# BadgerTechnologies/navigation

Measured on AMD Instinct MI355X. Metric: scored trajectories/sec (whole node) + costmap inflation cells/sec, 400x400 map, higher is better.
Workload: dtype f64

## Files before the change

navigation_amd/csrc/navgpu_fleet.h:

```cpp
#pragma once
#include <algorithm>
#include <cfloat>
#include <cmath>
#include <cstdio>
#include <cstdlib>
#include <cstring>
#include <ctime>
#include <mutex>
#include <string>
#include <vector>

#include "navgpu_device.h"

using namespace navgpu;

namespace navgpu {
extern thread_local std::string g_last_error;

#define HIP_TRY(expr)                                                                              \
  do {                                                                                             \
    hipError_t e_ = (expr);                                                                        \
    if (e_ != hipSuccess) {                                                                        \
      g_last_error = std::string(#expr) + ": " + hipGetErrorString(e_);                            \
      return NAVGPU_ERR_HIP;                                                                       \
    }                                                                                              \
  } while (0)

inline hipError_t waitStream(hipStream_t s) { return hipStreamSynchronize(s); }

struct EventPair {
  int kernel;
  hipEvent_t a, b;
};
int ensureCompleteGrids(navgpu_fleet* f, uint32_t first, uint32_t count);
}

struct navgpu_fleet {
  navgpu_fleet_desc desc{};
  std::recursive_mutex mu;
  hipStream_t stream = nullptr;
  CostmapDev cm{};
  PlannerDev pl{};
  bool planner_configured = false, inflation_configured = false, planner_staged = false;
  bool shift_pending = false;
  uint32_t shift_first = 0, shift_count = 0;
  std::vector<void*> allocs;
  std::vector<double> h_origin;
  std::vector<double> h_fp_spec;
  std::vector<uint32_t> h_fp_n;
  navgpu_inflation_params infl{};
  navgpu_obstacle_params obsp{};
  double fp_radius = 0.0;
  std::vector<void*> pinned;
  ObsCsr* hp_obs = nullptr;
  uint32_t *hp_cnt = nullptr, *hp_used = nullptr, *hp_plan_cnt = nullptr;
  float* hp_pts = nullptr;
  double *hp_fpw = nullptr, *hp_pose = nullptr, *hp_plan = nullptr, *hp_front = nullptr;
  int32_t *hp_shift = nullptr, *hp_align = nullptr;
  uint32_t *hp_reach = nullptr, *hp_fpn = nullptr;
  uint8_t *cm_stage_dev = nullptr, *cm_stage_host = nullptr, *pl_stage_dev = nullptr, *pl_stage_host = nullptr;
  size_t cm_stage_bytes = 0, pl_stage_bytes = 0;
  bool bounded_grids = true;
  std::vector<uint8_t> grid_partial;
  std::vector<int32_t> h_box;
  std::vector<uint64_t> inputs_gen, cycle_gen;
  void touchInputs(uint32_t first, uint32_t count) {
    for (uint32_t i = first; i < first + count && i < inputs_gen.size(); ++i) ++inputs_gen[i];
  }
  navgpu_robot_state* hp_state = nullptr;
  navgpu_plan_result* hp_result = nullptr;
  bool hp_dma_pending = false;
  int cycles_in_flight = 1;
  int res_slot = 0;
  hipEvent_t ev_cycle[2] = {nullptr, nullptr}, ev_cm_h2d = nullptr, ev_pl_h2d = nullptr;
  bool ev_cycle_set[2] = {false, false}, ev_cm_set = false, ev_pl_set = false;
  hipError_t waitMirrors(hipEvent_t ev, bool set) {
    if (cycles_in_flight < 2) return navgpu::waitStream(stream);
    return set ? hipEventSynchronize(ev) : hipSuccess;
  }
  struct LocalPlannerState {
    std::vector<double> plan;
    double T[3] = {0, 0, 0};
    bool has_T = false, have_plan = false;
    bool xy_tolerance_latch = false, rotating_to_goal = false;
  };
  std::vector<LocalPlannerState> lp;
  navgpu_local_limits lp_limits{};
  bool lp_configured = false;
  struct TpHost {
    std::vector<double> plan;
    double final_goal_x = 0, final_goal_y = 0;
    bool final_goal_position_valid = false;
    navgpu_tp_state st{};
    std::vector<navgpu_tp_sample> made;
    int n_points = 0;
  };
  TpDev tp{};
  bool tp_configured = false;
// ... 38 lines not shown
    return NAVGPU_OK;
  }
  template <class T>
  int allocPinned(T** p, size_t count) {
    void* q = nullptr;
    hipError_t e = hipHostMalloc(&q, std::max<size_t>(count * sizeof(T), 16), hipHostMallocDefault);
    if (e != hipSuccess) {
      g_last_error = std::string("hipHostMalloc: ") + hipGetErrorString(e);
      return NAVGPU_ERR_HIP;
    }
    memset(q, 0, std::max<size_t>(count * sizeof(T), 16));
    pinned.push_back(q);
    *p = static_cast<T*>(q);
    return NAVGPU_OK;
  }
  void release(void* q) {
    if (!q) return;
    auto it = std::find(allocs.begin(), allocs.end(), q);
    if (it != allocs.end()) allocs.erase(it);
    hipFree(q);
  }
  bool rangeOk(uint32_t first, uint32_t count) const { return count > 0 && first < desc.n_instances && count <= desc.n_instances - first; }

  int beginKernel(int k, EventPair* ep) {
    if (!profiling || !((prof_mask >> k) & 1u)) return NAVGPU_OK;
    if (free_events.empty()) {
      EventPair n{};
      HIP_TRY(hipEventCreate(&n.a));
      HIP_TRY(hipEventCreate(&n.b));
      free_events.push_back(n);
    }
    *ep = free_events.back();
    free_events.pop_back();
    ep->kernel = k;
    HIP_TRY(hipEventRecord(ep->a, stream));
    return NAVGPU_OK;
  }
  int endKernel(EventPair* ep) {
    if (!profiling || !ep->a) return NAVGPU_OK;
    HIP_TRY(hipEventRecord(ep->b, stream));
    events.push_back(*ep);
    if (events.size() > 8192) return foldEvents();
    return NAVGPU_OK;
  }
  int foldEvents() {
    if (events.empty()) return NAVGPU_OK;
    HIP_TRY(waitStream(stream));
    for (auto& e : events) {
      float ms = 0;
      HIP_TRY(hipEventElapsedTime(&ms, e.a, e.b));
      prof_ms[e.kernel] += ms;
      prof_n[e.kernel] += 1;
      free_events.push_back(e);
    }
    events.clear();
    return NAVGPU_OK;
  }
};

#ifndef NAVGPU_TEST_NO_FLEET_LOCK
struct FleetGuard {
  std::lock_guard<std::recursive_mutex> lk;
  explicit FleetGuard(navgpu_fleet* f) : lk(f->mu) { (void)hipSetDevice(f->desc.device); }
};
#else
struct FleetGuard {
  explicit FleetGuard(navgpu_fleet* f) { (void)hipSetDevice(f->desc.device); }
};
#endif

#define PROFILED(fleet, kid, launch_expr)            \
  do {                                               \
    EventPair ep_{};                                 \
    int rc_ = (fleet)->beginKernel((kid), &ep_);     \
    if (rc_) return rc_;                             \
    launch_expr;                                     \
    rc_ = (fleet)->endKernel(&ep_);                  \
    if (rc_) return rc_;                             \
  } while (0)

inline int checkLaunch() {
  hipError_t e = hipGetLastError();
  if (e != hipSuccess) {
    g_last_error = std::string("kernel launch: ") + hipGetErrorString(e);
    return NAVGPU_ERR_HIP;
  }
  return NAVGPU_OK;
}
```

navigation_amd/csrc/navgpu_host.cpp:

```cpp
#include "navgpu_fleet.h"

namespace navgpu {
thread_local std::string g_last_error;
}

extern "C" {

const char* navgpu_version(void) { return "navgpu 0.1 (gfx950)"; }
const char* navgpu_strerror(int status) {
  switch (status) {
    case NAVGPU_OK: return "ok";
    case NAVGPU_ERR_INVALID: return "invalid argument";
    case NAVGPU_ERR_NO_DEVICE: return "no usable HIP device (this library has no CPU fallback)";
    case NAVGPU_ERR_HIP: return "HIP runtime error";
    case NAVGPU_ERR_CAPACITY: return "input exceeds a capacity given at fleet creation";
    case NAVGPU_ERR_STATE: return "call sequence violated";
    default: return "unknown status";
  }
}
const char* navgpu_last_error(void) { return g_last_error.c_str(); }
int navgpu_device_count(void) {
  int n = 0;
  if (hipGetDeviceCount(&n) != hipSuccess) return 0;
  return n;
// ... 7 lines not shown
  if (!d || !out || d->n_instances == 0 || d->size_x == 0 || d->size_y == 0 || !(d->resolution > 0)) return NAVGPU_ERR_INVALID;
  if ((uint64_t)((d->size_x + 127) / 128) * ((d->size_y + 15) / 16) > 8192) {
    g_last_error = "navgpu_fleet_create: costmap larger than 16.7 M cells";
    return NAVGPU_ERR_CAPACITY;
  }
  if (d->max_footprint > (uint32_t)kMaxFootprint) return NAVGPU_ERR_CAPACITY;
  if ((uint64_t)d->size_x * d->size_y > (1ull << 30) || d->size_x > 65535 || d->size_y > 65535) return NAVGPU_ERR_CAPACITY;
  int ndev = 0;
  if (hipGetDeviceCount(&ndev) != hipSuccess || ndev <= 0 || d->device < 0 || d->device >= ndev) {
    g_last_error = "no HIP device";
    return NAVGPU_ERR_NO_DEVICE;
  }
  HIP_TRY(hipSetDevice(d->device));
  auto* f = new navgpu_fleet();
  f->desc = *d;
  if (f->desc.max_observations == 0) f->desc.max_observations = 1;
  if (f->desc.max_points == 0) f->desc.max_points = 1;
  if (f->desc.max_plan == 0) f->desc.max_plan = 1;
  if (f->desc.max_sim_steps == 0) f->desc.max_sim_steps = 64;
  const uint32_t n = d->n_instances;
  if (hipStreamCreateWithFlags(&f->stream, hipStreamNonBlocking) != hipSuccess) {
    g_last_error = "hipStreamCreate failed";
    delete f;
    return NAVGPU_ERR_NO_DEVICE;
  }
  CostmapDev& cm = f->cm;
  cm.nx = d->size_x;
  cm.ny = d->size_y;
  cm.cells = d->size_x * d->size_y;
  cm.cells_padded = (cm.cells + 63) & ~63u;
  cm.res = d->resolution;
  cm.layers = d->layers;
  cm.track_unknown = d->track_unknown;
  cm.master_default = d->track_unknown ? kNoInfo : kFree;
  cm.obstacle_default = d->track_unknown ? kNoInfo : kFree;
  cm.obs_enabled = 1;
  cm.footprint_clearing = 1;
  cm.combination_method = 1;
  cm.max_obstacle_height = 2.0;
  cm.z_voxels = 10;
  cm.unknown_threshold = 15;
  cm.mark_threshold = 0;
  cm.origin_z = 0.0;
  cm.z_resolution = 0.2;
  cm.max_obs = f->desc.max_observations;
  cm.max_points = f->desc.max_points;
// ... 81 lines not shown
  pl.inv_res = 1.0 / cm.res;
  pl.origin = cm.origin;
  pl.master = cm.master;
  pl.max_plan = f->desc.max_plan;
  pl.max_sim_steps = f->desc.max_sim_steps;
  {
    size_t off = 0;
    auto take = [&](size_t bytes) {
      const size_t at = off;
      off = (off + bytes + 255) & ~(size_t)255;
      return at;
    };
    const size_t o_state = take(sizeof(navgpu_robot_state) * n), o_front = take(sizeof(double) * 2 * n), o_align = take(sizeof(int32_t) * n),
                 o_reach = take(sizeof(uint32_t) * n), o_pcnt = take(sizeof(uint32_t) * n), o_plan = take(sizeof(double) * 2 * (size_t)n * pl.max_plan);
    f->pl_stage_bytes = off;
    uint8_t *d = nullptr, *h = nullptr;
    A(d, off);
    if ((rc = f->allocPinned(&h, off)) != 0) {
      navgpu_fleet_destroy(f);
      return rc;
    }
    f->pl_stage_dev = d;
    f->pl_stage_host = h;
    pl.state = reinterpret_cast<navgpu_robot_state*>(d + o_state);
    pl.front_last = reinterpret_cast<double*>(d + o_front);
    pl.align_on = reinterpret_cast<int32_t*>(d + o_align);
    pl.bfs_reach = reinterpret_cast<uint32_t*>(d + o_reach);
    pl.plan_count = reinterpret_cast<uint32_t*>(d + o_pcnt);
    pl.plan = reinterpret_cast<double*>(d + o_plan);
    f->hp_state = reinterpret_cast<navgpu_robot_state*>(h + o_state);
    f->hp_front = reinterpret_cast<double*>(h + o_front);
    f->hp_align = reinterpret_cast<int32_t*>(h + o_align);
    f->hp_reach = reinterpret_cast<uint32_t*>(h + o_reach);
    f->hp_plan_cnt = reinterpret_cast<uint32_t*>(h + o_pcnt);
    f->hp_plan = reinterpret_cast<double*>(h + o_plan);
  }
  A(pl.fp_spec, (size_t)n * kMaxFootprint * 2);
  A(pl.fp_n, n);
  A(pl.axis_count, (size_t)n * 4);
  A(pl.path, (size_t)n * pl.cells);
  A(pl.goal, (size_t)n * pl.cells);
  A(pl.goal_front, (size_t)n * pl.cells);
  if (bfs_scratch_words(cm.nx, cm.ny)) A(pl.bfs_scratch, (size_t)n * bfs_scratch_words(cm.nx, cm.ny));
  pl.bfs_grids = 3;
  pl.within = nullptr;
  A(pl.bfs_box, (size_t)n * 8);
// ... 23 lines not shown
  for (auto& s : st) {
    memset(&s, 0, sizeof(s));
    s.last_min_x = -FLT_MAX;
    s.last_min_y = -FLT_MAX;
    s.last_max_x = FLT_MAX;
    s.last_max_y = FLT_MAX;
  }
  hipError_t e = hipMemcpyAsync(cm.state, st.data(), sizeof(InstCostmapState) * n, hipMemcpyHostToDevice, f->stream);
  if (e == hipSuccess) e = hipMemsetAsync(pl.bfs_reach, 0, sizeof(uint32_t) * n, f->stream);
  if (e == hipSuccess) e = hipMemsetAsync(pl.bfs_levels, 0, sizeof(uint32_t) * 3 * n, f->stream);
  if (e == hipSuccess) e = waitStream(f->stream);
  if (e != hipSuccess || checkLaunch() != NAVGPU_OK) {
    if (e != hipSuccess) g_last_error = std::string("fleet init: ") + hipGetErrorString(e);
    navgpu_fleet_destroy(f);
    return NAVGPU_ERR_NO_DEVICE;
  }
  *out = f;
  return NAVGPU_OK;
}

int navgpu_fleet_destroy(navgpu_fleet* f) {
  if (!f) return NAVGPU_ERR_INVALID;
  if (f->stream) waitStream(f->stream);
  for (auto& e : f->events) {
    hipEventDestroy(e.a);
    hipEventDestroy(e.b);
  }
  for (auto& e : f->free_events) {
    hipEventDestroy(e.a);
    hipEventDestroy(e.b);
  }
  for (hipEvent_t e : {f->ev_cycle[0], f->ev_cycle[1], f->ev_cm_h2d, f->ev_pl_h2d})
    if (e) hipEventDestroy(e);
  for (void* p : f->allocs) hipFree(p);
  for (void* p : f->pinned) hipHostFree(p);
  if (f->stream) hipStreamDestroy(f->stream);
  delete f;
  return NAVGPU_OK;
}
int navgpu_sync(navgpu_fleet* f) {
  if (!f) return NAVGPU_ERR_INVALID;
  FleetGuard guard_(f);
  HIP_TRY(waitStream(f->stream));
  return NAVGPU_OK;
}
void* navgpu_stream(navgpu_fleet* f) { return f ? (void*)f->stream : nullptr; }
int navgpu_fleet_set_alloc_limit(navgpu_fleet* f, uint64_t max_bytes) {
  if (!f) return NAVGPU_ERR_INVALID;
  FleetGuard guard_(f);
  f->alloc_limit = (size_t)max_bytes;
  return NAVGPU_OK;
}

int navgpu_fleet_set_origin(navgpu_fleet* f, uint32_t first, uint32_t count, const double* xy) {
  if (!f || !xy || !f->rangeOk(first, count)) return NAVGPU_ERR_INVALID;
  FleetGuard guard_(f);
  f->touchInputs(first, count);
  memcpy(&f->h_origin[(size_t)first * 2], xy, sizeof(double) * 2 * count);
// ... 492 lines not shown
  if (e == hipSuccess) e = hipMemcpyAsync(f->pl.fp_n + first, &fp_n[first], sizeof(uint32_t) * count, hipMemcpyHostToDevice, f->stream);
  if (e == hipSuccess) e = waitStream(f->stream);
  if (e != hipSuccess) {
    if (fresh_prep) f->release(fresh_prep);
    g_last_error = std::string("navgpu_set_footprint: ") + hipGetErrorString(e);
    return NAVGPU_ERR_HIP;
  }
  f->h_fp_n.swap(fp_n);
  f->h_fp_spec.swap(fp_spec);
  f->fp_radius = fp_radius;
  if (f->planner_configured) {
    uint8_t* keep = fresh_prep ? fresh_prep : f->pl.prep;
    if (fresh_prep) f->release(f->pl.prep);
    f->pl = np;
    f->pl.prep = keep;
    f->pl.prep_stride = stride;
  }
  return NAVGPU_OK;
}

int navgpu_costmap_stage(navgpu_fleet* f, uint32_t first, uint32_t count, const double* poses, const navgpu_observation* obs,
                         uint32_t n_obs, const float* points, uint32_t n_points_total) {
  if (!f || !poses || !f->rangeOk(first, count) || (n_obs && (!obs || (!points && n_points_total)))) return NAVGPU_ERR_INVALID;
  FleetGuard guard_(f);
  CostmapDev& cm = f->cm;
  if (f->desc.rolling_window && f->shift_pending) return NAVGPU_ERR_STATE;
  if (f->desc.rolling_window) f->touchInputs(first, count);
  HIP_TRY(f->waitMirrors(f->ev_cm_h2d, f->ev_cm_set));
  for (uint32_t li = 0; li < count; ++li) f->hp_cnt[first + li] = f->hp_used[first + li] = 0;
  for (uint32_t k = 0; k < n_obs; ++k) {
    const navgpu_observation& o = obs[k];
    if (o.instance < first || o.instance >= first + count) return NAVGPU_ERR_INVALID;
    const uint32_t i = o.instance;
    if (f->hp_cnt[i] >= cm.max_obs || f->hp_used[i] + o.n_points > cm.max_points) return NAVGPU_ERR_CAPACITY;
    if ((uint64_t)o.first_point + o.n_points > n_points_total) return NAVGPU_ERR_INVALID;
    ObsCsr& d = f->hp_obs[(size_t)i * cm.max_obs + f->hp_cnt[i]++];
    d.first_point = f->hp_used[i];
    d.n_points = o.n_points;
    d.flags = o.flags;
    d.pad = 0;
    d.ox = o.origin_x;
    d.oy = o.origin_y;
    d.oz = o.origin_z;
    d.obstacle_range = o.obstacle_range;
    d.raytrace_range = o.raytrace_range;
    if (o.n_points)
      memcpy(&f->hp_pts[((size_t)i * cm.max_points + f->hp_used[i]) * 3], points + (size_t)o.first_point * 3, sizeof(float) * 3 * o.n_points);
// ... 50 lines not shown

static int applyPendingShift(navgpu_fleet* f, uint32_t first, uint32_t count) {
  CostmapDev& cm = f->cm;
  if (!(f->desc.rolling_window && f->shift_pending)) return NAVGPU_OK;
  if (first != f->shift_first || count != f->shift_count) return NAVGPU_ERR_STATE;
  if (first != 0 || count != f->desc.n_instances) return NAVGPU_ERR_INVALID;
  launch_shift_u8(cm.master, cm.master_alt, cm, first, count, cm.master_default, f->stream);
  std::swap(cm.master, cm.master_alt);
  f->pl.master = cm.master;
  if (cm.obst) {
    launch_shift_u8(cm.obst, cm.obst_alt, cm, first, count, cm.obstacle_default, f->stream);
    std::swap(cm.obst, cm.obst_alt);
  }
  if (cm.voxel) {
    launch_shift_u32(cm.voxel, cm.voxel_alt, cm, first, count, 0x0000FFFFu, f->stream);
    std::swap(cm.voxel, cm.voxel_alt);
  }
  f->shift_pending = false;
  return NAVGPU_OK;
}

int navgpu_costmap_update(navgpu_fleet* f, uint32_t first, uint32_t count) {
  if (!f || !f->rangeOk(first, count)) return NAVGPU_ERR_INVALID;
  FleetGuard guard_(f);
  f->touchInputs(first, count);
  CostmapDev& cm = f->cm;
  if ((cm.layers & NAVGPU_LAYER_INFLATION) && !f->inflation_configured) return NAVGPU_ERR_STATE;
  {
    int rc = applyPendingShift(f, first, count);
    if (rc) return rc;
  }
  PROFILED(f, NAVGPU_K_OBSTACLE, launch_obstacle(cm, first, count, nullptr, 0, f->stream));
  PROFILED(f, NAVGPU_K_MERGE, launch_merge(cm, first, count, nullptr, f->stream));
  if (cm.layers & NAVGPU_LAYER_INFLATION) PROFILED(f, NAVGPU_K_INFLATE, launch_inflate(cm, first, count, nullptr, f->stream));
  return checkLaunch();
}

int navgpu_costmap_bounds(navgpu_fleet* f, uint32_t first, uint32_t count, int32_t* boxes) {
  if (!f || !boxes || !f->rangeOk(first, count)) return NAVGPU_ERR_INVALID;
  FleetGuard guard_(f);
  std::vector<InstCostmapState> st(count);
  HIP_TRY(hipMemcpyAsync(st.data(), f->cm.state + first, sizeof(InstCostmapState) * count, hipMemcpyDeviceToHost, f->stream));
  HIP_TRY(waitStream(f->stream));
  for (uint32_t i = 0; i < count; ++i)
    for (int k = 0; k < 4; ++k) boxes[4 * i + k] = st[i].box[k];
  return NAVGPU_OK;
}
// ... 79 lines not shown
extern "C++" int navgpu::ensureCompleteGrids(navgpu_fleet* f, uint32_t first, uint32_t count) {
  if (NAVGPU_DEBUG_ENV("NAVGPU_DEBUG_RAW_GRIDS")) return NAVGPU_OK;
  for (uint32_t i = first; i < first + count; ++i)
    if (f->grid_partial[i] && f->cycle_gen[i] != f->inputs_gen[i]) {
      g_last_error = "MapGrids of instance " + std::to_string(i) + " were searched inside the robot's box only and the costmap / plan they came from has changed; "
                     "read them before the next update or call navgpu_planner_set_bounded_map_grids(f, 0)";
      return NAVGPU_ERR_STATE;
    }
  PlannerDev pl = f->pl;
  pl.bfs_bounded = 0;
  for (uint32_t i = first; i < first + count;) {
    if (!f->grid_partial[i]) {
      ++i;
      continue;
    }
    uint32_t j = i;
    while (j < first + count && f->grid_partial[j]) f->grid_partial[j++] = 0;
    launch_bfs(pl, i, j - i, f->stream);
    i = j;
  }
  return checkLaunch();
}

static int restageReach(navgpu_fleet* f) {
  if (!f->planner_staged) return NAVGPU_OK;
  PlannerDev& pl = f->pl;
  HIP_TRY(waitStream(f->stream));
  const uint32_t n = f->desc.n_instances;
  for (uint32_t i = 0; i < n; ++i) {
    const uint32_t np = f->hp_plan_cnt[i];
    if (!np) {
      f->hp_reach[i] = 0;
      continue;
    }
    const double* last = &f->hp_plan[((size_t)i * pl.max_plan + np - 1) * 2];
    f->hp_reach[i] = bfsReachCells(f, f->hp_state[i], last[0], last[1]);
  }
  HIP_TRY(hipMemcpyAsync(pl.bfs_reach, f->hp_reach, sizeof(uint32_t) * n, hipMemcpyHostToDevice, f->stream));
  f->hp_dma_pending = true;
  if (f->cycles_in_flight > 1) {
    HIP_TRY(hipEventRecord(f->ev_pl_h2d, f->stream));
    f->ev_pl_set = true;
  }
  return NAVGPU_OK;
}

int navgpu_planner_set_bounded_map_grids(navgpu_fleet* f, int32_t enable) {
  if (!f) return NAVGPU_ERR_INVALID;
  FleetGuard guard_(f);
  f->bounded_grids = enable != 0;
  return restageReach(f);
}
int navgpu_planner_set_map_grid_options(navgpu_fleet* f, int32_t critic, int32_t aggregation, double yshift) {
  if (!f || critic < 0 || critic > 3 || aggregation < 0 || aggregation > 2 || !std::isfinite(yshift)) return NAVGPU_ERR_INVALID;
  FleetGuard guard_(f);
  PlannerDev& pl = f->pl;
  pl.mg_agg[critic] = aggregation;
  pl.mg_yshift[critic] = yshift;
  pl.mg_generic = 0;
  for (int k = 0; k < 4; ++k)
    if (pl.mg_agg[k] != 0 || pl.mg_yshift[k] != 0.0) pl.mg_generic = 1;
// ... 22 lines not shown
  double steps;
  if (cfg.discretize_by_time)
    steps = ceil(cfg.sim_time / cfg.sim_granularity);
  else {
    double vmax = cfg.max_trans_vel >= 0 ? cfg.max_trans_vel + 1e-4
                                         : hypot(std::max(fabs(cfg.min_vel_x), fabs(cfg.max_vel_x)), std::max(fabs(cfg.min_vel_y), fabs(cfg.max_vel_y)));
    steps = ceil(std::max(vmax * cfg.sim_time / cfg.sim_granularity, fabs(cfg.max_rot_vel) * cfg.sim_time / cfg.angular_sim_granularity)) + 1;
  }
  if (steps > pl.max_sim_steps) {
    g_last_error = "max_sim_steps too small for this sim_time / granularity";
    return NAVGPU_ERR_CAPACITY;
  }
  const uint32_t nI = f->desc.n_instances;
  const uint32_t ax = (uint32_t)(std::max(cfg.vx_samples, 2) + 1), ay = (uint32_t)(std::max(cfg.vy_samples, 2) + 1),
                 at = (uint32_t)(std::max(cfg.vth_samples, 2) + 1);
  const uint32_t max_samples = ax * ay * at;
  const uint32_t score_blocks = 2 * ((max_samples + std::min(kScoreThreads, NAVGPU_SCORE_TAB_THREADS) - 1) / std::min(kScoreThreads, NAVGPU_SCORE_TAB_THREADS)) + at + 2;
  PlannerDev np = pl;
  np.cfg = cfg;
  np.scale_path = pl.res * cfg.path_distance_bias * 0.5;
  np.scale_goal = pl.res * cfg.goal_distance_bias * 0.5;
  np.scale_obstacle = pl.res * cfg.occdist_scale;
  const bool resize = max_axis != pl.max_axis || max_samples != pl.max_samples;
  float* n_axis = nullptr;
  double* n_part_cost = nullptr;
  int32_t* n_part_index = nullptr;
  double* n_sample_cost = nullptr;
  int32_t* n_sample_status = nullptr;
  uint8_t* n_prep = nullptr;
  uint32_t n_stride = pl.prep_stride;
  auto dropNew = [&] {
    f->release(n_axis);
    f->release(n_part_cost);
    f->release(n_part_index);
    f->release(n_sample_cost);
    f->release(n_sample_status);
    f->release(n_prep);
  };
  int rc = NAVGPU_OK;
  if (resize) {
    np.max_axis = max_axis;
    np.max_samples = max_samples;
    np.score_blocks = score_blocks;
    if (!rc) rc = f->alloc(&n_axis, (size_t)nI * 3 * max_axis);
    if (!rc) rc = f->alloc(&n_part_cost, (size_t)nI * score_blocks);
    if (!rc) rc = f->alloc(&n_part_index, (size_t)nI * score_blocks);
    if (!rc && f->desc.keep_sample_costs) rc = f->alloc(&n_sample_cost, (size_t)nI * max_samples);
    if (!rc && f->desc.keep_sample_costs) rc = f->alloc(&n_sample_status, (size_t)nI * max_samples);
  }
  if (!rc) {
    planWindow(f, np, f->h_fp_n, f->h_fp_spec, f->fp_radius);
    rc = allocPrep(f, np, &n_prep, &n_stride);
  }
  if (!rc && waitStream(f->stream) != hipSuccess) rc = NAVGPU_ERR_HIP;
  if (rc) {
    dropNew();
    return rc;
  }
  if (resize) {
    f->release(pl.axis_samples);
    f->release(pl.part_cost);
    f->release(pl.part_index);
    f->release(pl.sample_cost);
    f->release(pl.sample_status);
    np.axis_samples = n_axis;
    np.part_cost = n_part_cost;
    np.part_index = n_part_index;
    np.sample_cost = n_sample_cost;
    np.sample_status = n_sample_status;
  }
  if (n_prep) {
    f->release(pl.prep);
    np.prep = n_prep;
    np.prep_stride = n_stride;
  }
  pl = np;
  f->planner_configured = true;
  f->touchInputs(0, nI);
  if ((rc = restageReach(f)) != NAVGPU_OK) return rc;
  HIP_TRY(waitStream(f->stream));
  return NAVGPU_OK;
}

int navgpu_planner_set_plan(navgpu_fleet* f, uint32_t first, uint32_t count) {
  if (!f || !f->rangeOk(first, count)) return NAVGPU_ERR_INVALID;
  FleetGuard guard_(f);
  HIP_TRY(hipMemsetAsync(f->pl.osc_flags + first, 0, sizeof(uint32_t) * count, f->stream));
  return NAVGPU_OK;
}

int navgpu_planner_stage(navgpu_fleet* f, uint32_t first, uint32_t count, const navgpu_robot_state* states, const double* plan_xy,
                         uint32_t n_plan_total) {
  if (!f || !states || !plan_xy || !f->rangeOk(first, count)) return NAVGPU_ERR_INVALID;
  FleetGuard guard_(f);
  if (!f->planner_configured) return NAVGPU_ERR_STATE;
  PlannerDev& pl = f->pl;
  const navgpu_dwa_config& c = pl.cfg;
  for (uint32_t li = 0; li < count; ++li) {
    const navgpu_robot_state& s = states[li];
    if (s.plan_count == 0) return NAVGPU_ERR_INVALID;
    if (s.plan_count > pl.max_plan) return NAVGPU_ERR_CAPACITY;
    if ((uint64_t)s.plan_first + s.plan_count > n_plan_total) return NAVGPU_ERR_INVALID;
  }
  HIP_TRY(f->waitMirrors(f->ev_pl_h2d, f->ev_pl_set));
  for (uint32_t li = 0; li < count; ++li) {
    const uint32_t i = first + li;
    const navgpu_robot_state& s = states[li];
    f->hp_state[i] = s;
    memcpy(&f->hp_plan[(size_t)i * pl.max_plan * 2], plan_xy + (size_t)s.plan_first * 2, sizeof(double) * 2 * s.plan_count);
    f->hp_plan_cnt[i] = s.plan_count;
    const double gx = plan_xy[((size_t)s.plan_first + s.plan_count - 1) * 2], gy = plan_xy[((size_t)s.plan_first + s.plan_count - 1) * 2 + 1];
    const double sq_dist = (s.pos[0] - gx) * (s.pos[0] - gx) + (s.pos[1] - gy) * (s.pos[1] - gy);
    const double angle_to_goal = atan2(gy - s.pos[1], gx - s.pos[0]);
    f->hp_front[2 * i] = gx + c.forward_point_distance * cos(angle_to_goal);
    f->hp_front[2 * i + 1] = gy + c.forward_point_distance * sin(angle_to_goal);
    f->hp_align[i] = sq_dist > c.forward_point_distance * c.forward_point_distance * c.cheat_factor ? 1 : 0;
    f->hp_reach[i] = bfsReachCells(f, s, gx, gy);
  }
  f->touchInputs(first, count);
  if (first == 0 && count == f->desc.n_instances) {
    HIP_TRY(hipMemcpyAsync(f->pl_stage_dev, f->pl_stage_host, f->pl_stage_bytes, hipMemcpyHostToDevice, f->stream));
  } else {
    HIP_TRY(hipMemcpyAsync(pl.state + first, f->hp_state + first, sizeof(navgpu_robot_state) * count, hipMemcpyHostToDevice, f->stream));
    HIP_TRY(hipMemcpyAsync(pl.plan + (size_t)first * pl.max_plan * 2, f->hp_plan + (size_t)first * pl.max_plan * 2, sizeof(double) * 2 * (size_t)count * pl.max_plan, hipMemcpyHostToDevice, f->stream));
    HIP_TRY(hipMemcpyAsync(pl.plan_count + first, f->hp_plan_cnt + first, sizeof(uint32_t) * count, hipMemcpyHostToDevice, f->stream));
    HIP_TRY(hipMemcpyAsync(pl.front_last + (size_t)first * 2, f->hp_front + (size_t)first * 2, sizeof(double) * 2 * count, hipMemcpyHostToDevice, f->stream));
    HIP_TRY(hipMemcpyAsync(pl.align_on + first, f->hp_align + first, sizeof(int32_t) * count, hipMemcpyHostToDevice, f->stream));
    HIP_TRY(hipMemcpyAsync(pl.bfs_reach + first, f->hp_reach + first, sizeof(uint32_t) * count, hipMemcpyHostToDevice, f->stream));
  }
  if (f->cycles_in_flight > 1) {
    HIP_TRY(hipEventRecord(f->ev_pl_h2d, f->stream));
    f->ev_pl_set = true;
  }
  f->planner_staged = true;
  f->hp_dma_pending = true;
  return NAVGPU_OK;
}

int navgpu_planner_stage_poses(navgpu_fleet* f, uint32_t first, uint32_t count, const float* pos_xyth, const float* vel_xyth) {
  if (!f || !pos_xyth || !vel_xyth || !f->rangeOk(first, count)) return NAVGPU_ERR_INVALID;
  FleetGuard guard_(f);
  if (!f->planner_configured || !f->planner_staged) return NAVGPU_ERR_STATE;
  PlannerDev& pl = f->pl;
  const navgpu_dwa_config& c = pl.cfg;
  for (uint32_t i = first; i < first + count; ++i)
    if (!f->hp_plan_cnt[i]) {
      g_last_error = "navgpu_planner_stage_poses: instance " + std::to_string(i) + " has no staged plan";
      return NAVGPU_ERR_STATE;
    }
  if (f->hp_dma_pending) {
    HIP_TRY(f->waitMirrors(f->ev_pl_h2d, f->ev_pl_set));
    f->hp_dma_pending = false;
  }
  for (uint32_t li = 0; li < count; ++li) {
    const uint32_t i = first + li;
    navgpu_robot_state& s = f->hp_state[i];
    for (int k = 0; k < 3; ++k) {
      s.pos[k] = pos_xyth[3 * li + k];
      s.vel[k] = vel_xyth[3 * li + k];
    }
    const double* last = &f->hp_plan[((size_t)i * pl.max_plan + f->hp_plan_cnt[i] - 1) * 2];
    const double gx = last[0], gy = last[1];
    const double sq_dist = (s.pos[0] - gx) * (s.pos[0] - gx) + (s.pos[1] - gy) * (s.pos[1] - gy);
    const double angle_to_goal = atan2(gy - s.pos[1], gx - s.pos[0]);
    f->hp_front[2 * i] = gx + c.forward_point_distance * cos(angle_to_goal);
    f->hp_front[2 * i + 1] = gy + c.forward_point_distance * sin(angle_to_goal);
    f->hp_align[i] = sq_dist > c.forward_point_distance * c.forward_point_distance * c.cheat_factor ? 1 : 0;
    f->hp_reach[i] = bfsReachCells(f, s, gx, gy);
  }
  f->touchInputs(first, count);
  PoseChunk ch;
  ch.state = pl.state;
  ch.front_last = pl.front_last;
  ch.align_on = pl.align_on;
  ch.bfs_reach = pl.bfs_reach;
  for (uint32_t at = 0; at < count; at += kPoseChunk) {
    ch.first = first + at;
    ch.count = std::min(kPoseChunk, count - at);
    memcpy(ch.st, f->hp_state + ch.first, sizeof(navgpu_robot_state) * ch.count);
    memcpy(ch.front, f->hp_front + (size_t)ch.first * 2, sizeof(double) * 2 * ch.count);
    memcpy(ch.align, f->hp_align + ch.first, sizeof(int32_t) * ch.count);
    memcpy(ch.reach, f->hp_reach + ch.first, sizeof(uint32_t) * ch.count);
    launch_stage_poses(ch, f->stream);
  }
  return checkLaunch();
}

int navgpu_planner_wavefront_boxes(navgpu_fleet* f, uint32_t first, uint32_t count, int32_t* boxes) {
  if (!f || !boxes || !f->rangeOk(first, count)) return NAVGPU_ERR_INVALID;
  FleetGuard guard_(f);
  for (uint32_t li = 0; li < count; ++li) {
    const uint32_t i = first + li;
    if (f->grid_partial[i])
      memcpy(boxes + 4 * li, &f->h_box[(size_t)4 * i], sizeof(int32_t) * 4);
    else {
      boxes[4 * li] = 0;
      boxes[4 * li + 1] = (int32_t)f->pl.nx - 1;
      boxes[4 * li + 2] = 0;
      boxes[4 * li + 3] = (int32_t)f->pl.ny - 1;
    }
  }
  return NAVGPU_OK;
}

#ifdef NAVGPU_DEBUG_SWITCHES
extern "C" int navgpu_debug_prep_image(navgpu_fleet* f, uint32_t inst, uint8_t* out, uint32_t cap, uint32_t* win, uint32_t* bytes) {
  waitStream(f->stream);
  const uint32_t n = std::min<uint32_t>(cap, f->pl.prep_stride);
  hipMemcpy(out, f->pl.prep + (size_t)inst * f->pl.prep_stride, n, hipMemcpyDeviceToHost);
  *win = f->pl.win;
  *bytes = n;
  return 0;
}
#endif
int navgpu_planner_cycle(navgpu_fleet* f, uint32_t first, uint32_t count) {
  if (!f || !f->rangeOk(first, count)) return NAVGPU_ERR_INVALID;
  FleetGuard guard_(f);
  if (!f->planner_configured || !f->planner_staged) return NAVGPU_ERR_STATE;
  PlannerDev& pl = f->pl;
  const int prev_slot = f->res_slot;
  if (f->cycles_in_flight > 1) {
    if (first != 0 || count != f->desc.n_instances) return NAVGPU_ERR_STATE;
    pl.result = f->hp_result + (size_t)(prev_slot ^ 1) * f->desc.n_instances;
  }
  pl.bfs_bounded = 1;
  for (uint32_t i = first; i < first + count; ++i) {
    f->grid_partial[i] = robotBox(f, i, f->hp_state[i].pos, f->hp_reach[i], &f->h_box[(size_t)4 * i]) ? 1 : 0;
    f->cycle_gen[i] = f->inputs_gen[i];
  }
  launch_samples(pl, first, count, f->stream);
#ifdef NAVGPU_DEBUG_SWITCHES
  if (getenv("NAVGPU_DEBUG_BFS_TRACE") && !pl.bfs_trace) f->alloc(&pl.bfs_trace, (size_t)f->desc.n_instances * 3 * 8);
#endif
  PROFILED(f, NAVGPU_K_BFS, launch_bfs(pl, first, count, f->stream, pl.bfs_order + (size_t)first * 3, true));
#ifdef NAVGPU_DEBUG_SWITCHES
  if (pl.bfs_trace) {
    std::vector<unsigned long long> h((size_t)count * 24);
    hipMemcpyAsync(h.data(), pl.bfs_trace, h.size() * 8, hipMemcpyDeviceToHost, f->stream);
    waitStream(f->stream);
    if (FILE* fp = fopen(getenv("NAVGPU_DEBUG_BFS_TRACE"), "w")) {
      for (size_t i = 0; i < (size_t)count * 3; ++i)
        fprintf(fp, "%zu %llu %llu %llu %llu %llu %llu %llu %llu\n", i, h[8 * i], h[8 * i + 1] & 0xFFFFFFFFFFFFull, h[8 * i + 1] >> 48, h[8 * i + 2], h[8 * i + 3], h[8 * i + 4], h[8 * i + 5], h[8 * i + 6]);
      fclose(fp);
    }
  }
#endif
  uint32_t n_blocks = 0;
  PROFILED(f, NAVGPU_K_SCORE, n_blocks = launch_score(pl, first, count, nullptr, f->stream));
  PROFILED(f, NAVGPU_K_SELECT, launch_select(pl, first, count, n_blocks, f->stream));
  int rc = checkLaunch();
  if (f->cycles_in_flight > 1) {
    const int slot = prev_slot ^ 1;
    if (rc == NAVGPU_OK && hipEventRecord(f->ev_cycle[slot], f->stream) != hipSuccess) rc = NAVGPU_ERR_HIP;
    if (rc == NAVGPU_OK) {
      f->res_slot = slot;
      f->ev_cycle_set[slot] = true;
    } else {
      pl.result = f->hp_result + (size_t)prev_slot * f->desc.n_instances;
    }
  }
  return rc;
}

int navgpu_planner_set_cycles_in_flight(navgpu_fleet* f, int32_t cycles) {
  if (!f || cycles < 1 || cycles > 2) return NAVGPU_ERR_INVALID;
  FleetGuard guard_(f);
  HIP_TRY(waitStream(f->stream));
  if (cycles > 1)
    for (hipEvent_t* e : {&f->ev_cycle[0], &f->ev_cycle[1], &f->ev_cm_h2d, &f->ev_pl_h2d})
      if (!*e) HIP_TRY(hipEventCreateWithFlags(e, hipEventDisableTiming));
  if (cycles == 1 && f->res_slot) {
    memcpy(f->hp_result, f->hp_result + f->desc.n_instances, sizeof(navgpu_plan_result) * f->desc.n_instances);
    f->res_slot = 0;
    f->pl.result = f->hp_result;
  }
  f->ev_cycle_set[0] = f->ev_cycle_set[1] = f->ev_cm_set = f->ev_pl_set = false;
  f->cycles_in_flight = cycles;
  return NAVGPU_OK;
}

int navgpu_planner_results_previous(navgpu_fleet* f, uint32_t first, uint32_t count, navgpu_plan_result* results) {
  if (!f || !results || !f->rangeOk(first, count)) return NAVGPU_ERR_INVALID;
  FleetGuard guard_(f);
  const int slot = f->res_slot ^ 1;
  if (f->cycles_in_flight < 2 || !f->ev_cycle_set[slot]) return NAVGPU_ERR_STATE;
  HIP_TRY(hipEventSynchronize(f->ev_cycle[slot]));
  memcpy(results, f->hp_result + (size_t)slot * f->desc.n_instances + first, sizeof(navgpu_plan_result) * count);
  return NAVGPU_OK;
}

int navgpu_planner_results(navgpu_fleet* f, uint32_t first, uint32_t count, navgpu_plan_result* results) {
  if (!f || !results || !f->rangeOk(first, count)) return NAVGPU_ERR_INVALID;
  FleetGuard guard_(f);
  HIP_TRY(waitStream(f->stream));
  memcpy(results, f->hp_result + (size_t)f->res_slot * f->desc.n_instances + first, sizeof(navgpu_plan_result) * count);
  return NAVGPU_OK;
}

int navgpu_planner_trajectory(navgpu_fleet* f, uint32_t instance, double* xyth, uint32_t cap) {
  if (!f || !xyth || instance >= f->desc.n_instances) return NAVGPU_ERR_INVALID;
  FleetGuard guard_(f);
  HIP_TRY(waitStream(f->stream));
  const navgpu_plan_result r = f->hp_result[(size_t)f->res_slot * f->desc.n_instances + instance];
  uint32_t n = std::min<uint32_t>(r.n_points > 0 ? r.n_points : 0, cap);
  if (n) {
    HIP_TRY(hipMemcpyAsync(xyth, f->pl.traj + (size_t)instance * f->pl.max_sim_steps * 3, sizeof(double) * 3 * n, hipMemcpyDeviceToHost, f->stream));
// ... 153 lines not shown
```

Measured before the change: 5.653 billion.

## Run score/select on a second stream with double-buffered planner state

Adds a second HIP stream and a duplicated set of per-cycle planner buffers (staged state, BFS grids, axis samples, and a costmap master snapshot). When two cycles are in flight, the score and select kernels run on the back stream while the front stream stages the next cycle, with events joining the two. The aim is to overlap host staging and costmap work with trajectory scoring. In exchange it uses much more device memory, adds a device-to-device snapshot copy of the master grid every cycle, and brings considerable synchronisation complexity.

```diff
diff --git a/navigation_amd/csrc/navgpu_fleet.h b/navigation_amd/csrc/navgpu_fleet.h
--- a/navigation_amd/csrc/navgpu_fleet.h
+++ b/navigation_amd/csrc/navgpu_fleet.h
@@ -14,6 +14,8 @@
 
 using namespace navgpu;
 
+#pragma weak hipStreamWaitEvent
+
 namespace navgpu {
 extern thread_local std::string g_last_error;
 
@@ -27,6 +29,21 @@
   } while (0)
 
 inline hipError_t waitStream(hipStream_t s) { return hipStreamSynchronize(s); }
+inline bool haveStreamWaitEvent() { return &hipStreamWaitEvent != nullptr; }
+inline hipError_t streamWaitEvent(hipStream_t s, hipEvent_t e) { return hipStreamWaitEvent(s, e, 0); }
+
+struct CycleSet {
+  uint8_t* stage_head = nullptr;
+  navgpu_robot_state* state = nullptr;
+  double* front_last = nullptr;
+  int32_t* align_on = nullptr;
+  uint32_t* bfs_reach = nullptr;
+  float* axis_samples = nullptr;
+  int32_t* axis_count = nullptr;
+  int32_t* counters = nullptr;
+  uint32_t *path = nullptr, *goal = nullptr, *goal_front = nullptr;
+  uint8_t* master_snap = nullptr;
+};
 
 struct EventPair {
   int kernel;
@@ -39,6 +56,7 @@
   navgpu_fleet_desc desc{};
   std::recursive_mutex mu;
   hipStream_t stream = nullptr;
+  hipStream_t stream_back = nullptr;
   CostmapDev cm{};
   PlannerDev pl{};
   bool planner_configured = false, inflation_configured = false, planner_staged = false;
@@ -74,6 +92,36 @@
   int res_slot = 0;
   hipEvent_t ev_cycle[2] = {nullptr, nullptr}, ev_cm_h2d = nullptr, ev_pl_h2d = nullptr;
   bool ev_cycle_set[2] = {false, false}, ev_cm_set = false, ev_pl_set = false;
+  CycleSet alt{};
+  bool two_streams = false;
+  bool alt_fresh = false;
+  bool back_ahead = false;
+  hipEvent_t ev_front = nullptr, ev_join = nullptr;
+  void swapSets() {
+    std::swap(pl.state, alt.state);
+    std::swap(pl.front_last, alt.front_last);
+    std::swap(pl.align_on, alt.align_on);
+    std::swap(pl.bfs_reach, alt.bfs_reach);
+    std::swap(pl.axis_samples, alt.axis_samples);
+    std::swap(pl.axis_count, alt.axis_count);
+    std::swap(pl.counters, alt.counters);
+    std::swap(pl.path, alt.path);
+    std::swap(pl.goal, alt.goal);
+    std::swap(pl.goal_front, alt.goal_front);
+    std::swap(cur_stage_head, alt.stage_head);
+    std::swap(cur_master_snap, alt.master_snap);
+  }
+  uint8_t *cur_stage_head = nullptr, *cur_master_snap = nullptr;
+  size_t stage_head_bytes = 0;
+  size_t o_front = 0, o_align = 0, o_reach = 0;
+  hipError_t joinBack() {
+    if (!back_ahead) return hipSuccess;
+    back_ahead = false;
+    hipError_t e = hipEventRecord(ev_join, stream_back);
+    if (e == hipSuccess) e = navgpu::streamWaitEvent(stream, ev_join);
+    if (e != hipSuccess) e = navgpu::waitStream(stream_back);
+    return e;
+  }
   hipError_t waitMirrors(hipEvent_t ev, bool set) {
     if (cycles_in_flight < 2) return navgpu::waitStream(stream);
     return set ? hipEventSynchronize(ev) : hipSuccess;
@@ -158,7 +206,7 @@
   }
   bool rangeOk(uint32_t first, uint32_t count) const { return count > 0 && first < desc.n_instances && count <= desc.n_instances - first; }
 
-  int beginKernel(int k, EventPair* ep) {
+  int beginKernel(int k, EventPair* ep, hipStream_t on = nullptr) {
     if (!profiling || !((prof_mask >> k) & 1u)) return NAVGPU_OK;
     if (free_events.empty()) {
       EventPair n{};
@@ -169,12 +217,12 @@
     *ep = free_events.back();
     free_events.pop_back();
     ep->kernel = k;
-    HIP_TRY(hipEventRecord(ep->a, stream));
-    return NAVGPU_OK;
-  }
-  int endKernel(EventPair* ep) {
+    HIP_TRY(hipEventRecord(ep->a, on ? on : stream));
+    return NAVGPU_OK;
+  }
+  int endKernel(EventPair* ep, hipStream_t on = nullptr) {
     if (!profiling || !ep->a) return NAVGPU_OK;
-    HIP_TRY(hipEventRecord(ep->b, stream));
+    HIP_TRY(hipEventRecord(ep->b, on ? on : stream));
     events.push_back(*ep);
     if (events.size() > 8192) return foldEvents();
     return NAVGPU_OK;
@@ -182,6 +230,7 @@
   int foldEvents() {
     if (events.empty()) return NAVGPU_OK;
     HIP_TRY(waitStream(stream));
+    if (stream_back) HIP_TRY(waitStream(stream_back));
     for (auto& e : events) {
       float ms = 0;
       HIP_TRY(hipEventElapsedTime(&ms, e.a, e.b));
@@ -195,25 +244,34 @@
 };
 
 #ifndef NAVGPU_TEST_NO_FLEET_LOCK
+enum GuardKind { kJoined, kPipelined };
 struct FleetGuard {
   std::lock_guard<std::recursive_mutex> lk;
-  explicit FleetGuard(navgpu_fleet* f) : lk(f->mu) { (void)hipSetDevice(f->desc.device); }
+  explicit FleetGuard(navgpu_fleet* f, GuardKind kind = kJoined) : lk(f->mu) {
+    (void)hipSetDevice(f->desc.device);
+    if (kind == kJoined) (void)f->joinBack();
+  }
 };
 #else
+enum GuardKind { kJoined, kPipelined };
 struct FleetGuard {
-  explicit FleetGuard(navgpu_fleet* f) { (void)hipSetDevice(f->desc.device); }
+  explicit FleetGuard(navgpu_fleet* f, GuardKind kind = kJoined) {
+    (void)hipSetDevice(f->desc.device);
+    if (kind == kJoined) (void)f->joinBack();
+  }
 };
 #endif
 
-#define PROFILED(fleet, kid, launch_expr)            \
-  do {                                               \
-    EventPair ep_{};                                 \
-    int rc_ = (fleet)->beginKernel((kid), &ep_);     \
-    if (rc_) return rc_;                             \
-    launch_expr;                                     \
-    rc_ = (fleet)->endKernel(&ep_);                  \
-    if (rc_) return rc_;                             \
+#define PROFILED_ON(fleet, on, kid, launch_expr)         \
+  do {                                                   \
+    EventPair ep_{};                                     \
+    int rc_ = (fleet)->beginKernel((kid), &ep_, (on));   \
+    if (rc_) return rc_;                                 \
+    launch_expr;                                         \
+    rc_ = (fleet)->endKernel(&ep_, (on));                \
+    if (rc_) return rc_;                                 \
   } while (0)
+#define PROFILED(fleet, kid, launch_expr) PROFILED_ON(fleet, nullptr, kid, launch_expr)
 
 inline int checkLaunch() {
   hipError_t e = hipGetLastError();
diff --git a/navigation_amd/csrc/navgpu_host.cpp b/navigation_amd/csrc/navgpu_host.cpp
--- a/navigation_amd/csrc/navgpu_host.cpp
+++ b/navigation_amd/csrc/navgpu_host.cpp
@@ -53,6 +53,11 @@
   if (hipStreamCreateWithFlags(&f->stream, hipStreamNonBlocking) != hipSuccess) {
     g_last_error = "hipStreamCreate failed";
     delete f;
+    return NAVGPU_ERR_NO_DEVICE;
+  }
+  if (haveStreamWaitEvent() && hipStreamCreateWithFlags(&f->stream_back, hipStreamNonBlocking) != hipSuccess) {
+    g_last_error = "hipStreamCreate failed";
+    navgpu_fleet_destroy(f);
     return NAVGPU_ERR_NO_DEVICE;
   }
   CostmapDev& cm = f->cm;
@@ -180,6 +185,11 @@
     }
     f->pl_stage_dev = d;
     f->pl_stage_host = h;
+    f->cur_stage_head = d;
+    f->stage_head_bytes = o_pcnt;
+    f->o_front = o_front;
+    f->o_align = o_align;
+    f->o_reach = o_reach;
     pl.state = reinterpret_cast<navgpu_robot_state*>(d + o_state);
     pl.front_last = reinterpret_cast<double*>(d + o_front);
     pl.align_on = reinterpret_cast<int32_t*>(d + o_align);
@@ -249,6 +259,7 @@
 int navgpu_fleet_destroy(navgpu_fleet* f) {
   if (!f) return NAVGPU_ERR_INVALID;
   if (f->stream) waitStream(f->stream);
+  if (f->stream_back) waitStream(f->stream_back);
   for (auto& e : f->events) {
     hipEventDestroy(e.a);
     hipEventDestroy(e.b);
@@ -257,10 +268,11 @@
     hipEventDestroy(e.a);
     hipEventDestroy(e.b);
   }
-  for (hipEvent_t e : {f->ev_cycle[0], f->ev_cycle[1], f->ev_cm_h2d, f->ev_pl_h2d})
+  for (hipEvent_t e : {f->ev_cycle[0], f->ev_cycle[1], f->ev_cm_h2d, f->ev_pl_h2d, f->ev_front, f->ev_join})
     if (e) hipEventDestroy(e);
   for (void* p : f->allocs) hipFree(p);
   for (void* p : f->pinned) hipHostFree(p);
+  if (f->stream_back) hipStreamDestroy(f->stream_back);
   if (f->stream) hipStreamDestroy(f->stream);
   delete f;
   return NAVGPU_OK;
@@ -799,7 +811,7 @@
 int navgpu_costmap_stage(navgpu_fleet* f, uint32_t first, uint32_t count, const double* poses, const navgpu_observation* obs,
                          uint32_t n_obs, const float* points, uint32_t n_points_total) {
   if (!f || !poses || !f->rangeOk(first, count) || (n_obs && (!obs || (!points && n_points_total)))) return NAVGPU_ERR_INVALID;
-  FleetGuard guard_(f);
+  FleetGuard guard_(f, f->desc.rolling_window ? kJoined : kPipelined);
   CostmapDev& cm = f->cm;
   if (f->desc.rolling_window && f->shift_pending) return NAVGPU_ERR_STATE;
   if (f->desc.rolling_window) f->touchInputs(first, count);
@@ -896,7 +908,7 @@
 
 int navgpu_costmap_update(navgpu_fleet* f, uint32_t first, uint32_t count) {
   if (!f || !f->rangeOk(first, count)) return NAVGPU_ERR_INVALID;
-  FleetGuard guard_(f);
+  FleetGuard guard_(f, f->desc.rolling_window ? kJoined : kPipelined);
   f->touchInputs(first, count);
   CostmapDev& cm = f->cm;
   if ((cm.layers & NAVGPU_LAYER_INFLATION) && !f->inflation_configured) return NAVGPU_ERR_STATE;
@@ -1022,6 +1034,12 @@
   return checkLaunch();
 }
 
+static hipError_t freshenAlt(navgpu_fleet* f) {
+  if (f->alt_fresh) return hipSuccess;
+  f->alt_fresh = true;
+  return hipMemcpyAsync(f->alt.stage_head, f->cur_stage_head, f->stage_head_bytes, hipMemcpyDeviceToDevice, f->stream);
+}
+
 static int restageReach(navgpu_fleet* f) {
   if (!f->planner_staged) return NAVGPU_OK;
   PlannerDev& pl = f->pl;
@@ -1036,7 +1054,8 @@
     const double* last = &f->hp_plan[((size_t)i * pl.max_plan + np - 1) * 2];
     f->hp_reach[i] = bfsReachCells(f, f->hp_state[i], last[0], last[1]);
   }
-  HIP_TRY(hipMemcpyAsync(pl.bfs_reach, f->hp_reach, sizeof(uint32_t) * n, hipMemcpyHostToDevice, f->stream));
+  if (f->two_streams) HIP_TRY(freshenAlt(f));
+  HIP_TRY(hipMemcpyAsync(f->two_streams ? f->alt.bfs_reach : pl.bfs_reach, f->hp_reach, sizeof(uint32_t) * n, hipMemcpyHostToDevice, f->stream));
   f->hp_dma_pending = true;
   if (f->cycles_in_flight > 1) {
     HIP_TRY(hipEventRecord(f->ev_pl_h2d, f->stream));
@@ -1105,7 +1124,7 @@
   np.scale_goal = pl.res * cfg.goal_distance_bias * 0.5;
   np.scale_obstacle = pl.res * cfg.occdist_scale;
   const bool resize = max_axis != pl.max_axis || max_samples != pl.max_samples;
-  float* n_axis = nullptr;
+  float *n_axis = nullptr, *n_axis_alt = nullptr;
   double* n_part_cost = nullptr;
   int32_t* n_part_index = nullptr;
   double* n_sample_cost = nullptr;
@@ -1114,6 +1133,7 @@
   uint32_t n_stride = pl.prep_stride;
   auto dropNew = [&] {
     f->release(n_axis);
+    f->release(n_axis_alt);
     f->release(n_part_cost);
     f->release(n_part_index);
     f->release(n_sample_cost);
@@ -1126,6 +1146,7 @@
     np.max_samples = max_samples;
     np.score_blocks = score_blocks;
     if (!rc) rc = f->alloc(&n_axis, (size_t)nI * 3 * max_axis);
+    if (!rc && f->two_streams) rc = f->alloc(&n_axis_alt, (size_t)nI * 3 * max_axis);
     if (!rc) rc = f->alloc(&n_part_cost, (size_t)nI * score_blocks);
     if (!rc) rc = f->alloc(&n_part_index, (size_t)nI * score_blocks);
     if (!rc && f->desc.keep_sample_costs) rc = f->alloc(&n_sample_cost, (size_t)nI * max_samples);
@@ -1147,6 +1168,10 @@
     f->release(pl.sample_cost);
     f->release(pl.sample_status);
     np.axis_samples = n_axis;
+    if (f->two_streams) {
+      f->release(f->alt.axis_samples);
+      f->alt.axis_samples = n_axis_alt;
+    }
     np.part_cost = n_part_cost;
     np.part_index = n_part_index;
     np.sample_cost = n_sample_cost;
@@ -1175,7 +1200,7 @@
 int navgpu_planner_stage(navgpu_fleet* f, uint32_t first, uint32_t count, const navgpu_robot_state* states, const double* plan_xy,
                          uint32_t n_plan_total) {
   if (!f || !states || !plan_xy || !f->rangeOk(first, count)) return NAVGPU_ERR_INVALID;
-  FleetGuard guard_(f);
+  FleetGuard guard_(f, kPipelined);
   if (!f->planner_configured) return NAVGPU_ERR_STATE;
   PlannerDev& pl = f->pl;
   const navgpu_dwa_config& c = pl.cfg;
@@ -1201,15 +1226,29 @@
     f->hp_reach[i] = bfsReachCells(f, s, gx, gy);
   }
   f->touchInputs(first, count);
+  const bool two = f->two_streams;
+  uint8_t* head = two ? f->alt.stage_head : f->cur_stage_head;
+  navgpu_robot_state* d_state = two ? f->alt.state : pl.state;
+  double* d_front = two ? f->alt.front_last : pl.front_last;
+  int32_t* d_align = two ? f->alt.align_on : pl.align_on;
+  uint32_t* d_reach = two ? f->alt.bfs_reach : pl.bfs_reach;
   if (first == 0 && count == f->desc.n_instances) {
-    HIP_TRY(hipMemcpyAsync(f->pl_stage_dev, f->pl_stage_host, f->pl_stage_bytes, hipMemcpyHostToDevice, f->stream));
+    if (head == f->pl_stage_dev) {
+      HIP_TRY(hipMemcpyAsync(f->pl_stage_dev, f->pl_stage_host, f->pl_stage_bytes, hipMemcpyHostToDevice, f->stream));
+    } else {
+      HIP_TRY(hipMemcpyAsync(head, f->pl_stage_host, f->stage_head_bytes, hipMemcpyHostToDevice, f->stream));
+      HIP_TRY(hipMemcpyAsync(f->pl_stage_dev + f->stage_head_bytes, f->pl_stage_host + f->stage_head_bytes, f->pl_stage_bytes - f->stage_head_bytes,
+                             hipMemcpyHostToDevice, f->stream));
+    }
+    if (two) f->alt_fresh = true;
   } else {
-    HIP_TRY(hipMemcpyAsync(pl.state + first, f->hp_state + first, sizeof(navgpu_robot_state) * count, hipMemcpyHostToDevice, f->stream));
+    if (two) HIP_TRY(freshenAlt(f));
+    HIP_TRY(hipMemcpyAsync(d_state + first, f->hp_state + first, sizeof(navgpu_robot_state) * count, hipMemcpyHostToDevice, f->stream));
     HIP_TRY(hipMemcpyAsync(pl.plan + (size_t)first * pl.max_plan * 2, f->hp_plan + (size_t)first * pl.max_plan * 2, sizeof(double) * 2 * (size_t)count * pl.max_plan, hipMemcpyHostToDevice, f->stream));
     HIP_TRY(hipMemcpyAsync(pl.plan_count + first, f->hp_plan_cnt + first, sizeof(uint32_t) * count, hipMemcpyHostToDevice, f->stream));
-    HIP_TRY(hipMemcpyAsync(pl.front_last + (size_t)first * 2, f->hp_front + (size_t)first * 2, sizeof(double) * 2 * count, hipMemcpyHostToDevice, f->stream));
-    HIP_TRY(hipMemcpyAsync(pl.align_on + first, f->hp_align + first, sizeof(int32_t) * count, hipMemcpyHostToDevice, f->stream));
-    HIP_TRY(hipMemcpyAsync(pl.bfs_reach + first, f->hp_reach + first, sizeof(uint32_t) * count, hipMemcpyHostToDevice, f->stream));
+    HIP_TRY(hipMemcpyAsync(d_front + (size_t)first * 2, f->hp_front + (size_t)first * 2, sizeof(double) * 2 * count, hipMemcpyHostToDevice, f->stream));
+    HIP_TRY(hipMemcpyAsync(d_align + first, f->hp_align + first, sizeof(int32_t) * count, hipMemcpyHostToDevice, f->stream));
+    HIP_TRY(hipMemcpyAsync(d_reach + first, f->hp_reach + first, sizeof(uint32_t) * count, hipMemcpyHostToDevice, f->stream));
   }
   if (f->cycles_in_flight > 1) {
     HIP_TRY(hipEventRecord(f->ev_pl_h2d, f->stream));
@@ -1222,7 +1261,7 @@
 
 int navgpu_planner_stage_poses(navgpu_fleet* f, uint32_t first, uint32_t count, const float* pos_xyth, const float* vel_xyth) {
   if (!f || !pos_xyth || !vel_xyth || !f->rangeOk(first, count)) return NAVGPU_ERR_INVALID;
-  FleetGuard guard_(f);
+  FleetGuard guard_(f, kPipelined);
   if (!f->planner_configured || !f->planner_staged) return NAVGPU_ERR_STATE;
   PlannerDev& pl = f->pl;
   const navgpu_dwa_config& c = pl.cfg;
@@ -1253,10 +1292,16 @@
   }
   f->touchInputs(first, count);
   PoseChunk ch;
-  ch.state = pl.state;
-  ch.front_last = pl.front_last;
-  ch.align_on = pl.align_on;
-  ch.bfs_reach = pl.bfs_reach;
+  if (f->two_streams) {
+    if (first == 0 && count == f->desc.n_instances)
+      f->alt_fresh = true;
+    else
+      HIP_TRY(freshenAlt(f));
+  }
+  ch.state = f->two_streams ? f->alt.state : pl.state;
+  ch.front_last = f->two_streams ? f->alt.front_last : pl.front_last;
+  ch.align_on = f->two_streams ? f->alt.align_on : pl.align_on;
+  ch.bfs_reach = f->two_streams ? f->alt.bfs_reach : pl.bfs_reach;
   for (uint32_t at = 0; at < count; at += kPoseChunk) {
     ch.first = first + at;
     ch.count = std::min(kPoseChunk, count - at);
@@ -1271,7 +1316,7 @@
 
 int navgpu_planner_wavefront_boxes(navgpu_fleet* f, uint32_t first, uint32_t count, int32_t* boxes) {
   if (!f || !boxes || !f->rangeOk(first, count)) return NAVGPU_ERR_INVALID;
-  FleetGuard guard_(f);
+  FleetGuard guard_(f, kPipelined);
   for (uint32_t li = 0; li < count; ++li) {
     const uint32_t i = first + li;
     if (f->grid_partial[i])
@@ -1298,13 +1343,21 @@
 #endif
 int navgpu_planner_cycle(navgpu_fleet* f, uint32_t first, uint32_t count) {
   if (!f || !f->rangeOk(first, count)) return NAVGPU_ERR_INVALID;
-  FleetGuard guard_(f);
+  FleetGuard guard_(f, kPipelined);
   if (!f->planner_configured || !f->planner_staged) return NAVGPU_ERR_STATE;
   PlannerDev& pl = f->pl;
   const int prev_slot = f->res_slot;
+  const bool two = f->two_streams;
+  hipStream_t back = two ? f->stream_back : f->stream;
   if (f->cycles_in_flight > 1) {
     if (first != 0 || count != f->desc.n_instances) return NAVGPU_ERR_STATE;
     pl.result = f->hp_result + (size_t)(prev_slot ^ 1) * f->desc.n_instances;
+  }
+  if (two) {
+    HIP_TRY(freshenAlt(f));
+    f->swapSets();
+    f->alt_fresh = false;
+    HIP_TRY(hipMemcpyAsync(f->cur_master_snap, f->cm.master, (size_t)f->desc.n_instances * pl.cells_padded, hipMemcpyDeviceToDevice, f->stream));
   }
   pl.bfs_bounded = 1;
   for (uint32_t i = first; i < first + count; ++i) {
@@ -1329,20 +1382,85 @@
   }
 #endif
   uint32_t n_blocks = 0;
-  PROFILED(f, NAVGPU_K_SCORE, n_blocks = launch_score(pl, first, count, nullptr, f->stream));
-  PROFILED(f, NAVGPU_K_SELECT, launch_select(pl, first, count, n_blocks, f->stream));
+  PlannerDev bp = pl;
+  if (two) {
+    bp.master = f->cur_master_snap;
+    f->back_ahead = true;
+    HIP_TRY(hipEventRecord(f->ev_front, f->stream));
+    HIP_TRY(streamWaitEvent(back, f->ev_front));
+  }
+  PROFILED_ON(f, back, NAVGPU_K_SCORE, n_blocks = launch_score(bp, first, count, nullptr, back));
+  PROFILED_ON(f, back, NAVGPU_K_SELECT, launch_select(bp, first, count, n_blocks, back));
   int rc = checkLaunch();
   if (f->cycles_in_flight > 1) {
     const int slot = prev_slot ^ 1;
-    if (rc == NAVGPU_OK && hipEventRecord(f->ev_cycle[slot], f->stream) != hipSuccess) rc = NAVGPU_ERR_HIP;
+    if (rc == NAVGPU_OK && hipEventRecord(f->ev_cycle[slot], back) != hipSuccess) rc = NAVGPU_ERR_HIP;
+    if (rc == NAVGPU_OK && two && f->ev_cycle_set[prev_slot] && streamWaitEvent(f->stream, f->ev_cycle[prev_slot]) != hipSuccess) rc = NAVGPU_ERR_HIP;
     if (rc == NAVGPU_OK) {
       f->res_slot = slot;
       f->ev_cycle_set[slot] = true;
     } else {
       pl.result = f->hp_result + (size_t)prev_slot * f->desc.n_instances;
+      if (two) {
+        waitStream(f->stream);
+        waitStream(back);
+        f->back_ahead = false;
+        f->swapSets();
+        f->alt_fresh = true;
+      }
     }
   }
   return rc;
+}
+
+static int allocSecondSet(navgpu_fleet* f) {
+  PlannerDev& pl = f->pl;
+  const size_t n = f->desc.n_instances;
+  CycleSet t;
+  uint8_t* snap = nullptr;
+  int rc = f->alloc(&t.stage_head, f->stage_head_bytes);
+  if (!rc && pl.axis_samples) rc = f->alloc(&t.axis_samples, n * 3 * pl.max_axis);
+  if (!rc) rc = f->alloc(&t.axis_count, n * 4);
+  if (!rc) rc = f->alloc(&t.counters, n * 2);
+  if (!rc) rc = f->alloc(&t.path, n * pl.cells);
+  if (!rc) rc = f->alloc(&t.goal, n * pl.cells);
+  if (!rc) rc = f->alloc(&t.goal_front, n * pl.cells);
+  if (!rc) rc = f->alloc(&t.master_snap, n * pl.cells_padded);
+  if (!rc) rc = f->alloc(&snap, n * pl.cells_padded);
+  if (!rc && waitStream(f->stream) != hipSuccess) rc = NAVGPU_ERR_HIP;
+  if (rc) {
+    for (void* q : {(void*)t.stage_head, (void*)t.axis_samples, (void*)t.axis_count, (void*)t.counters, (void*)t.path, (void*)t.goal, (void*)t.goal_front,
+                    (void*)t.master_snap, (void*)snap})
+      f->release(q);
+    return rc;
+  }
+  t.state = reinterpret_cast<navgpu_robot_state*>(t.stage_head);
+  t.front_last = reinterpret_cast<double*>(t.stage_head + f->o_front);
+  t.align_on = reinterpret_cast<int32_t*>(t.stage_head + f->o_align);
+  t.bfs_reach = reinterpret_cast<uint32_t*>(t.stage_head + f->o_reach);
+  f->alt = t;
+  f->cur_master_snap = snap;
+  return NAVGPU_OK;
+}
+static int dropSecondSet(navgpu_fleet* f) {
+  PlannerDev& pl = f->pl;
+  if (f->alt_fresh) HIP_TRY(hipMemcpy(f->cur_stage_head, f->alt.stage_head, f->stage_head_bytes, hipMemcpyDeviceToDevice));
+  if (f->cur_stage_head != f->pl_stage_dev) {
+    HIP_TRY(hipMemcpy(f->alt.stage_head, f->cur_stage_head, f->stage_head_bytes, hipMemcpyDeviceToDevice));
+    std::swap(f->cur_stage_head, f->alt.stage_head);
+    std::swap(pl.state, f->alt.state);
+    std::swap(pl.front_last, f->alt.front_last);
+    std::swap(pl.align_on, f->alt.align_on);
+    std::swap(pl.bfs_reach, f->alt.bfs_reach);
+  }
+  for (void* q : {(void*)f->alt.stage_head, (void*)f->alt.axis_samples, (void*)f->alt.axis_count, (void*)f->alt.counters, (void*)f->alt.path,
+                  (void*)f->alt.goal, (void*)f->alt.goal_front, (void*)f->alt.master_snap, (void*)f->cur_master_snap})
+    f->release(q);
+  f->alt = CycleSet{};
+  f->cur_master_snap = nullptr;
+  f->two_streams = false;
+  f->alt_fresh = false;
+  return NAVGPU_OK;
 }
 
 int navgpu_planner_set_cycles_in_flight(navgpu_fleet* f, int32_t cycles) {
@@ -1350,8 +1468,18 @@
   FleetGuard guard_(f);
   HIP_TRY(waitStream(f->stream));
   if (cycles > 1)
-    for (hipEvent_t* e : {&f->ev_cycle[0], &f->ev_cycle[1], &f->ev_cm_h2d, &f->ev_pl_h2d})
+    for (hipEvent_t* e : {&f->ev_cycle[0], &f->ev_cycle[1], &f->ev_cm_h2d, &f->ev_pl_h2d, &f->ev_front, &f->ev_join})
       if (!*e) HIP_TRY(hipEventCreateWithFlags(e, hipEventDisableTiming));
+  if (cycles > 1 && f->stream_back && !f->two_streams) {
+    int rc = allocSecondSet(f);
+    if (rc) return rc;
+    f->two_streams = true;
+    f->alt_fresh = false;
+  }
+  if (cycles == 1 && f->two_streams) {
+    int rc = dropSecondSet(f);
+    if (rc) return rc;
+  }
   if (cycles == 1 && f->res_slot) {
     memcpy(f->hp_result, f->hp_result + f->desc.n_instances, sizeof(navgpu_plan_result) * f->desc.n_instances);
     f->res_slot = 0;
@@ -1364,7 +1492,7 @@
 
 int navgpu_planner_results_previous(navgpu_fleet* f, uint32_t first, uint32_t count, navgpu_plan_result* results) {
   if (!f || !results || !f->rangeOk(first, count)) return NAVGPU_ERR_INVALID;
-  FleetGuard guard_(f);
+  FleetGuard guard_(f, kPipelined);
   const int slot = f->res_slot ^ 1;
   if (f->cycles_in_flight < 2 || !f->ev_cycle_set[slot]) return NAVGPU_ERR_STATE;
   HIP_TRY(hipEventSynchronize(f->ev_cycle[slot]));
```

After: 3.465 billion. -38.7%, worse.
